# EveryVoiceTTS/FastSpeech2_lightning

Hardware: AMD Instinct MI355X
Metric: mel-frames/sec (train fwd+bwd+optimizer, whole job) (higher is better)
Workload: dtype f32

## Files before the change

### fastspeech2_lightning_amd/csrc/gemm.hip

```cpp
#include <cstdlib>

#include <string.h>

#include "gemm_common.h"

namespace {

constexpr int BK = 16;
constexpr int LDS_PAD = 4;

template <int BM, int BN>
struct Tile {
  static constexpr int TM = BM / 64;
  static constexpr int TN = BN / 64;
  static constexpr int LDA = BM + LDS_PAD;
  static constexpr int LDB = BN + LDS_PAD;
  static constexpr int A_F4 = BM * BK / 4 / 256;
  static constexpr int B_F4 = BN * BK / 4 / 256;
};

template <int ROWS, int NF4>
__device__ __forceinline__ void load_tile(float4 (&reg)[NF4], const float* __restrict__ src, int ld,
                                          bool kcontig, int row0, int nrows, int k0, int klimit,
                                          int shift, int T, bool shift_rows, bool shift_k, int tid) {
// ... 237 lines not shown
      p.Rper = a.R / a.taps;
      if (a.Mc % a.T) return FS2HIP_EINVAL;
    } else {
      if (a.a_kcontig || a.b_kcontig || a.R % a.T) return FS2HIP_EINVAL;
    }
  }
  if (a.splitk > 1 && (a.a_kcontig || a.b_kcontig || !a.workspace)) return FS2HIP_EINVAL;
  if (a.colsum && (a.a_kcontig || a.b_kcontig)) return FS2HIP_EINVAL;
  if (a.splitk <= 1) a.counters = nullptr;
  if (a.counters && (long long)a.taps * ((a.Mc + 63) / 64) * ((a.Nc + 63) / 64) > FS2_SPLITK_COUNTERS) return FS2HIP_EINVAL;
  if (a.epi == FS2_EPI_RESID && !a.resid) return FS2HIP_EINVAL;
  if (a.epi == FS2_EPI_DACT && !a.aux) return FS2HIP_EINVAL;
  {
    auto fits = [&](long long ld) { return 4LL * a.Mc * ld < 0x7fffffffLL; };
    if (!fits(a.splitk > 1 ? a.Nc : a.ldc) || (a.out_pre && !fits(a.ldpre)) ||
        (a.epi == FS2_EPI_RESID && !fits(a.ldr)) || (a.epi == FS2_EPI_DACT && !fits(a.ldaux)))
      return FS2HIP_EINVAL;
  }
  p.drop = fs2_make_drop(a.drop_p, a.drop_seed, a.drop_step);
  int chunk = (a.R + a.splitk - 1) / a.splitk;
  p.r_chunk = ((chunk + BK - 1) / BK) * BK;
  const int nz = (a.shift_operand == 1 ? a.taps : 1) * a.splitk;
  static const int env_tile = getenv("FS2_GEMM_TILE") ? atoi(getenv("FS2_GEMM_TILE")) : 0;
  int tile = a.tile ? a.tile : env_tile;
  const bool v2_ok = a.a_kcontig || !a.b_kcontig;
  const bool v1_ok = !(a.taps > 1 && a.shift_operand == 0 && (p.Rper % BK));
  if (tile == 0) {
    const bool narrow = a.Nc <= 64 || (a.Nc % 128 != 0 && a.Nc % 128 <= 64) ||
                        ((long long)((a.Mc + 127) / 128) * ((a.Nc + 127) / 128) * nz < 384);
    const bool odd_taps = a.taps > 1 && (a.shift_operand == 0 ? (p.Rper % 32) != 0 : a.T < 32);
    tile = v2_ok ? (odd_taps ? (v1_ok && !a.operand_bf16 && !a.colsum ? 3 : 7) : (narrow ? 5 : 4)) : (narrow ? 2 : 1);
  }
  if (a.operand_bf16 == 3 && (tile < 4 || tile > 9)) return FS2HIP_EINVAL;
  if (tile >= 4) {
    if (tile != 32 && !v2_ok) return FS2HIP_EINVAL;
    route = {ROUTE_V2, tile, nz};
    return 0;
  }
  if (!v1_ok || a.colsum) return FS2HIP_EINVAL;
  route = {ROUTE_V1, tile, nz};
  return 0;
}

int gemm_launch(GemmP& p, const GemmRoute& route, hipStream_t s) {
  const Fs2GemmArgs& a = p.a;
  const int tile = route.tile, nz = route.nz;
  if (route.core == ROUTE_B) {
    if (tile == 33) return fs2_gemmws4_launch(p, s);
    if (tile >= 30) return fs2_gemmws_launch(p, tile, s);
    return fs2_gemmb_launch(p, tile, nz, s);
  }
  if (route.core == ROUTE_V2) {
    if (tile == 32) return fs2_gemmws32_launch(p, s);
    return tile >= 10 ? fs2_gemm2p_launch(p, tile, nz, s) : fs2_gemm2_launch(p, tile, nz, s);
  }
  if (tile == 3) {
    p.tiles_n = (a.Nc + 63) / 64;
    dim3 grid(((a.Mc + 63) / 64) * p.tiles_n, 1, nz);
    gemm_kernel<64, 64><<<grid, dim3(256), 0, s>>>(p);
  } else if (tile == 2) {
    p.tiles_n = (a.Nc + 63) / 64;
    dim3 grid(((a.Mc + 127) / 128) * p.tiles_n, 1, nz);
    gemm_kernel<128, 64><<<grid, dim3(256), 0, s>>>(p);
  } else {
    p.tiles_n = (a.Nc + 127) / 128;
    dim3 grid(((a.Mc + 127) / 128) * p.tiles_n, 1, nz);
    gemm_kernel<128, 128><<<grid, dim3(256), 0, s>>>(p);
  }
  FS2_LAUNCH_CHECK();
  return 0;
}
}

extern "C" int fs2hip_gemm(const Fs2GemmArgs* args, void* stream) {
  if (!args) return FS2HIP_EINVAL;
  GemmP p;
  GemmRoute route;
  const int rc = gemm_prepare(args, p, route);
  if (rc != 0) return rc;
  return gemm_launch(p, route, (hipStream_t)stream);
}

extern "C" int fs2hip_gemm_grouped(const Fs2GemmArgs* args, int n, void* stream) {
  if (!args || n < 1 || n > FS2_GEMM_GROUP_MAX) return FS2HIP_EINVAL;
  if (n == 1) return fs2hip_gemm(args, stream);
  GemmPG g;
  memset(&g, 0, sizeof(g));
  g.n = n;
  const bool stored = args[0].operand_bf16 == 4;
  int tile = args[0].tile;
  if (tile == 0) tile = stored ? 23 : 7;
  for (int i = 0; i < n; ++i) {
    Fs2GemmArgs m = args[i];
    if (m.operand_bf16 != args[0].operand_bf16 || (m.operand_bf16 != 0 && m.operand_bf16 != 4)) return FS2HIP_EINVAL;
    if ((m.a_kcontig != 0) != (args[0].a_kcontig != 0) || (m.b_kcontig != 0) != (args[0].b_kcontig != 0)) return FS2HIP_EINVAL;
    if (m.taps > 1 || m.counters || m.drop_p > 0.f) return FS2HIP_EINVAL;
    m.tile = tile;
    GemmRoute route;
    const int rc = gemm_prepare(&m, g.m[i], route);
    if (rc != 0) return rc;
    if (route.core != (stored ? ROUTE_B : ROUTE_V2) || route.tile != tile || route.nz != g.m[i].a.splitk) return FS2HIP_EINVAL;
  }
  return stored ? fs2_gemmb_launch_grouped(g, tile, (hipStream_t)stream) : fs2_gemm2_launch_grouped(g, tile, (hipStream_t)stream);
}
```

### fastspeech2_lightning_amd/csrc/gemm2.hip

```cpp
#include "gemm2_core.h"
namespace {

template <int BM, int BN, bool AKC, bool BKC, int NST, int TAPS, int BF>
__device__ __forceinline__ void gemm2_body(const GemmP& p, const int bid, const int nblk) {
  constexpr int TM = BM / 64, TN = BN / 64;
  constexpr int A_TILE = BM * BK2, B_TILE = BN * BK2, STAGE = A_TILE + B_TILE;
  constexpr int L = BM / 32 + BN / 32;
  static_assert(NST >= 2 && NST <= 4 && (NST - 2) * L < 64, "ring depth");
  __shared__ __attribute__((aligned(16))) float lds[NST * STAGE];
  const Fs2GemmArgs& a = p.a;
  const int tid = threadIdx.x, lane = tid & 63;
  const int wave = __builtin_amdgcn_readfirstlane(tid >> 6);
  const int wm = wave >> 1, wn = wave & 1;
  const int ntile = p.tiles_m * p.tiles_n;
  const int unit = fs2_xcd_remap(bid, nblk);
  const int z = unit / ntile;
  const int wg = unit - z * ntile;
  const int tile_m = wg / p.tiles_n, tile_n = wg - tile_m * p.tiles_n;
  const int m0 = tile_m * BM, n0 = tile_n * BN;

  int tapz = 0, split = 0;
  if (a.shift_operand == 1 || a.splitk > 1) {
    const int ntap = a.shift_operand == 1 ? a.taps : 1;
    split = z / ntap;
// ... 108 lines not shown
      else return FS2HIP_EINVAL;
    } else if (mode == TAPS_RED) FS2_GO(true, true, TAPS_RED);
    else if (mode == TAPS_NONE) FS2_GO(true, true, TAPS_NONE);
    else return FS2HIP_EINVAL;
  } else if (a.a_kcontig && !a.b_kcontig) {
    if (mode == TAPS_RED) FS2_GO(true, false, TAPS_RED);
    else if (mode == TAPS_NONE) FS2_GO(true, false, TAPS_NONE);
    else return FS2HIP_EINVAL;
  } else if (!a.a_kcontig && !a.b_kcontig) {
    if (mode == TAPS_ROWS) FS2_GO(false, false, TAPS_ROWS);
    else if (mode == TAPS_NONE) FS2_GO(false, false, TAPS_NONE);
    else return FS2HIP_EINVAL;
  } else {
    return FS2HIP_EINVAL;
  }
  FS2_LAUNCH_CHECK();
  return 0;
}

#undef FS2_GO

template <int BM, int BN, int NST>
int launch_grouped(GemmPG& g, hipStream_t s) {
  long long total = 0;
  for (int i = 0; i < g.n; ++i) {
    GemmP& p = g.m[i];
    const Fs2GemmArgs& a = p.a;
    const int chunk = (a.R + a.splitk - 1) / a.splitk;
    p.r_chunk = ((chunk + BK2 - 1) / BK2) * BK2;
    p.tiles_m = (a.Mc + BM - 1) / BM;
    p.tiles_n = (a.Nc + BN - 1) / BN;
    if (!fs2_gemm2_offsets_fit(a)) return FS2HIP_EINVAL;
    g.start[i] = (int)total;
    total += (long long)p.tiles_m * p.tiles_n * a.splitk;
    if (total > 0x7fffffffLL) return FS2HIP_EINVAL;
  }
  for (int i = g.n; i <= FS2_GEMM_GROUP_MAX; ++i) g.start[i] = (int)total;
  const Fs2GemmArgs& a = g.m[0].a;
  dim3 grid((unsigned)total), block(256);
  if (a.a_kcontig && a.b_kcontig) gemm2g_kernel<BM, BN, true, true, NST><<<grid, block, 0, s>>>(g);
  else if (a.a_kcontig && !a.b_kcontig) gemm2g_kernel<BM, BN, true, false, NST><<<grid, block, 0, s>>>(g);
  else if (!a.a_kcontig && !a.b_kcontig) gemm2g_kernel<BM, BN, false, false, NST><<<grid, block, 0, s>>>(g);
  else return FS2HIP_EINVAL;
  FS2_LAUNCH_CHECK();
  return 0;
}

}

int fs2_gemm2_launch_grouped(GemmPG& g, int tile, hipStream_t s) {
  switch (tile) {
    case 7: return launch_grouped<64, 64, 2>(g, s);
    case 8: return launch_grouped<128, 64, 2>(g, s);
    default: return FS2HIP_EINVAL;
  }
}

int fs2_gemm2_launch(GemmP& p, int tile, int nz, hipStream_t s) {
  const Fs2GemmArgs& a = p.a;
  const int chunk = (a.R + a.splitk - 1) / a.splitk;
  p.r_chunk = ((chunk + BK2 - 1) / BK2) * BK2;
  if (!fs2_gemm2_offsets_fit(a)) return FS2HIP_EINVAL;
  switch (tile) {
    case 4: return launch_tile<128, 128, 3, false>(p, nz, s);
    case 5: return launch_tile<128, 64, 3, false>(p, nz, s);
    case 6: return launch_tile<64, 64, 4, false>(p, nz, s);
    case 7: return launch_tile<64, 64, 2, true>(p, nz, s);
    case 8: return launch_tile<128, 64, 2, false>(p, nz, s);
    case 9: return launch_tile<128, 128, 2, false>(p, nz, s);
    default: return FS2HIP_EINVAL;
  }
}
```

### fastspeech2_lightning_amd/csrc/gemm_common.h

```cpp
#pragma once
#include "common.h"

struct GemmP {
  Fs2GemmArgs a;
  int Rper;
  int tiles_m;
  int tiles_n;
  int r_chunk;
  int probe;
  int staged;
  Fs2Drop drop;
};

struct GemmPG {
  int n;
  int start[FS2_GEMM_GROUP_MAX + 1];
  GemmP m[FS2_GEMM_GROUP_MAX];
};
__device__ __forceinline__ int fs2_group_member(const GemmPG& g, int bid) {
  int i = 0;
#pragma unroll
  for (int k = 1; k < FS2_GEMM_GROUP_MAX; ++k) i += (k < g.n && bid >= g.start[k]) ? 1 : 0;
  return i;
}

constexpr int FS2_EPI_OOB = (int)0x80000000;

__device__ __forceinline__ __amdgpu_buffer_rsrc_t fs2_epi_rsrc(const float* base, int rows, int ld) {
  return __builtin_amdgcn_make_buffer_rsrc((void*)base, 0, rows * ld * 4, 0x00020000);
}
__device__ __forceinline__ float fs2_buf_load(__amdgpu_buffer_rsrc_t r, int voff, int soff) {
  return __builtin_bit_cast(float, __builtin_amdgcn_raw_buffer_load_b32(r, voff, soff, 0));
}
__device__ __forceinline__ void fs2_buf_store(__amdgpu_buffer_rsrc_t r, int voff, int soff, float v) {
  __builtin_amdgcn_raw_buffer_store_b32(__builtin_bit_cast(unsigned, v), r, voff, soff, 0);
}
constexpr int FS2_SC1 = 16;
__device__ __forceinline__ void fs2_buf_store_sc1(__amdgpu_buffer_rsrc_t r, int voff, int soff, float v) {
  __builtin_amdgcn_raw_buffer_store_b32(__builtin_bit_cast(unsigned, v), r, voff, soff, FS2_SC1);
}

template <int BM, int BN, int EPI>
__device__ __forceinline__ void gemm_epilogue_impl(const GemmP& p, const f32x16 (&acc)[BM / 64][BN / 64], float* C,
                                                   int ldc, int m0, int n0, int wm, int wn, int lane) {
  constexpr int TM = BM / 64, TN = BN / 64;
  const Fs2GemmArgs& a = p.a;
  const Fs2Drop drop = fs2_resolve_drop(p.drop);
  const int mrow = m0 + wm * (BM / 2) + 4 * (lane >> 5);
  const __amdgpu_buffer_rsrc_t rc = fs2_epi_rsrc(C, a.Mc, ldc);
#define FS2_ROWOFF(i, r) ((i) * 32 + ((r) & 3) + 8 * ((r) >> 2))
#pragma unroll
  for (int j = 0; j < TN; ++j) {
    const int n = n0 + wn * (BN / 2) + j * 32 + (lane & 31);
    const bool col = n < a.Nc;
    const float bias = (EPI >= 0 && a.bias && col) ? a.bias[n] : 0.f;
    const int vc = col ? (mrow * ldc + n) * 4 : FS2_EPI_OOB;
#pragma unroll
    for (int i = 0; i < TM; ++i) {
      float v[16];
#pragma unroll
      for (int r = 0; r < 16; ++r) v[r] = acc[i][j][r];
      if (EPI >= 0) {
#pragma unroll
        for (int r = 0; r < 16; ++r) v[r] = a.alpha * v[r] + bias;
      }
      if (EPI == FS2_EPI_ACT) {
        if (a.out_pre) {
          const __amdgpu_buffer_rsrc_t rp = fs2_epi_rsrc(a.out_pre, a.Mc, a.ldpre);
          const int vp = col ? (mrow * a.ldpre + n) * 4 : FS2_EPI_OOB;
#pragma unroll
          for (int r = 0; r < 16; ++r) fs2_buf_store(rp, vp, FS2_ROWOFF(i, r) * a.ldpre * 4, v[r]);
        }
        if (a.act == FS2_ACT_RELU) {
#pragma unroll
          for (int r = 0; r < 16; ++r) v[r] = fs2_act(FS2_ACT_RELU, v[r]);
        } else if (a.act == FS2_ACT_SILU) {
#pragma unroll
          for (int r = 0; r < 16; ++r) v[r] = fs2_act(FS2_ACT_SILU, v[r]);
        } else if (a.act == FS2_ACT_TANH) {
#pragma unroll
          for (int r = 0; r < 16; ++r) v[r] = fs2_act(FS2_ACT_TANH, v[r]);
        }
      } else if (EPI == FS2_EPI_DACT) {
        const __amdgpu_buffer_rsrc_t rx = fs2_epi_rsrc(a.aux, a.Mc, a.ldaux);
        const int vx = col ? (mrow * a.ldaux + n) * 4 : FS2_EPI_OOB;
        float x[16];
#pragma unroll
        for (int r = 0; r < 16; ++r) x[r] = fs2_buf_load(rx, vx, FS2_ROWOFF(i, r) * a.ldaux * 4);
        if (a.act == FS2_ACT_RELU) {
#pragma unroll
          for (int r = 0; r < 16; ++r) v[r] *= fs2_dact(FS2_ACT_RELU, x[r]);
        } else if (a.act == FS2_ACT_SILU) {
#pragma unroll
          for (int r = 0; r < 16; ++r) v[r] *= fs2_dact(FS2_ACT_SILU, x[r]);
        } else if (a.act == FS2_ACT_TANH) {
#pragma unroll
          for (int r = 0; r < 16; ++r) v[r] *= fs2_dact(FS2_ACT_TANH, x[r]);
        }
      }
      if (EPI > 0 && drop.on) {
        if ((ldc & 1) == 0) {
          const int par = lane & 1;
          const unsigned he = (unsigned)((mrow * ldc + n) + par * ldc);
          const unsigned sh = par << 4;
#pragma unroll
          for (int r = 0; r < 16; r += 2) {
            const uint32_t H = fs2_hash32_lo(drop.seed, (he + (unsigned)(FS2_ROWOFF(i, r) * ldc)) >> 1);
            const uint32_t Hn = (uint32_t)__builtin_amdgcn_mov_dpp((int)H, 0xB1, 0xF, 0xF, true);
            const uint32_t ha = par ? Hn : H, hb = par ? H : Hn;
            v[r] *= ((ha >> sh) & 0xffffu) < drop.thresh ? 0.f : drop.scale;
            v[r + 1] *= ((hb >> sh) & 0xffffu) < drop.thresh ? 0.f : drop.scale;
          }
        } else {
#pragma unroll
          for (int r = 0; r < 16; ++r)
            v[r] *= fs2_drop_factor(drop, (unsigned long long)((unsigned)(vc + FS2_ROWOFF(i, r) * ldc * 4) >> 2));
        }
      }
      if (EPI == FS2_EPI_RESID) {
        const __amdgpu_buffer_rsrc_t rx = fs2_epi_rsrc(a.resid, a.Mc, a.ldr);
        const int vx = col ? (mrow * a.ldr + n) * 4 : FS2_EPI_OOB;
        float x[16];
#pragma unroll
        for (int r = 0; r < 16; ++r) x[r] = fs2_buf_load(rx, vx, FS2_ROWOFF(i, r) * a.ldr * 4);
#pragma unroll
        for (int r = 0; r < 16; ++r) v[r] = x[r] + a.res_scale * v[r];
      }
      if (EPI == -2) {
#pragma unroll
        for (int r = 0; r < 16; ++r) fs2_buf_store_sc1(rc, vc, FS2_ROWOFF(i, r) * ldc * 4, v[r]);
      } else {
#pragma unroll
        for (int r = 0; r < 16; ++r) fs2_buf_store(rc, vc, FS2_ROWOFF(i, r) * ldc * 4, v[r]);
      }
    }
  }
#undef FS2_ROWOFF
}

template <int BM, int BN>
__device__ __forceinline__ void splitk_finish(const GemmP& p, int m0, int n0, int tapz) {
  const Fs2GemmArgs& a = p.a;
  __shared__ int last_one;
  const int slot = (tapz * ((a.Mc + BM - 1) / BM) + m0 / BM) * p.tiles_n + n0 / BN;
  asm volatile("s_waitcnt vmcnt(0)" ::: "memory");
  __syncthreads();
  if (threadIdx.x == 0)
    last_one = __hip_atomic_fetch_add(a.counters + slot, 1, __ATOMIC_RELAXED, __HIP_MEMORY_SCOPE_AGENT) == a.splitk - 1;
  __syncthreads();
  if (!last_one) return;
  const long long slab = (long long)a.Mc * a.Nc;
  const long long kstride = (long long)a.taps * slab;
  const __amdgpu_buffer_rsrc_t rw = __builtin_amdgcn_make_buffer_rsrc((void*)(a.workspace + (long long)tapz * slab), 0, 0x7ffffffc, 0x00020000);
  float* C = a.C + (a.shift_operand == 1 ? (long long)tapz * a.c_tap_stride : 0);
  const bool vec = (a.Nc % 4) == 0 && (a.ldc % 4) == 0 && ((uintptr_t)C % 16) == 0 && ((uintptr_t)a.workspace % 16) == 0;
  constexpr int C4 = BN / 4;
  for (int e = threadIdx.x; e < BM * C4; e += blockDim.x) {
    const int m = m0 + e / C4, n = n0 + (e % C4) * 4;
    if (m >= a.Mc || n >= a.Nc) continue;
    const int off = (m * a.Nc + n) * 4;
    if (vec) {
      f32x4 t = {0.f, 0.f, 0.f, 0.f};
      for (int k0 = 0; k0 < a.splitk; k0 += 8) {
        f32x4 v[8];
#pragma unroll
        for (int u = 0; u < 8; ++u) {
          const __amdgpu_buffer_rsrc_t rk = __builtin_amdgcn_make_buffer_rsrc(
              (void*)(a.workspace + (long long)tapz * slab + (k0 + u) * kstride), 0, k0 + u < a.splitk ? 0x7ffffffc : 0, 0x00020000);
          v[u] = __builtin_bit_cast(f32x4, __builtin_amdgcn_raw_buffer_load_b128(rk, off, 0, FS2_SC1));
        }
        if (k0 == 0) {
          t = v[0];
#pragma unroll
          for (int u = 1; u < 8; ++u)
            if (u < a.splitk) t += v[u];
        } else {
#pragma unroll
          for (int u = 0; u < 8; ++u)
            if (k0 + u < a.splitk) t += v[u];
        }
      }
      *reinterpret_cast<f32x4*>(C + (long long)m * a.ldc + n) = t;
    } else {
      for (int i = 0; i < 4 && n + i < a.Nc; ++i) {
        float t = __builtin_bit_cast(float, __builtin_amdgcn_raw_buffer_load_b32(rw, off + 4 * i, 0, FS2_SC1));
        for (int k = 1; k < a.splitk; ++k) {
          const __amdgpu_buffer_rsrc_t rk = __builtin_amdgcn_make_buffer_rsrc(
              (void*)(a.workspace + (long long)tapz * slab + k * kstride), 0, 0x7ffffffc, 0x00020000);
          t += __builtin_bit_cast(float, __builtin_amdgcn_raw_buffer_load_b32(rk, off + 4 * i, 0, FS2_SC1));
        }
        C[(long long)m * a.ldc + n + i] = t;
      }
    }
  }
  if (threadIdx.x == 0) __hip_atomic_store(a.counters + slot, 0, __ATOMIC_RELAXED, __HIP_MEMORY_SCOPE_AGENT);
}

template <int BM, int BN>
__device__ __forceinline__ void gemm_epilogue(const GemmP& p, const f32x16 (&acc)[BM / 64][BN / 64], int m0, int n0,
                                              int wm, int wn, int lane, int split, int tapz) {
  const Fs2GemmArgs& a = p.a;
  float* C = a.C;
  if (a.splitk > 1) {
    C = a.workspace + ((long long)split * a.taps + tapz) * ((long long)a.Mc * a.Nc);
    if (a.counters) {
      gemm_epilogue_impl<BM, BN, -2>(p, acc, C, a.Nc, m0, n0, wm, wn, lane);
      splitk_finish<BM, BN>(p, m0, n0, tapz);
    } else {
      gemm_epilogue_impl<BM, BN, -1>(p, acc, C, a.Nc, m0, n0, wm, wn, lane);
    }
    return;
  }
  if (a.shift_operand == 1) C += (long long)tapz * a.c_tap_stride;
  switch (a.epi) {
    case FS2_EPI_ACT: gemm_epilogue_impl<BM, BN, FS2_EPI_ACT>(p, acc, C, a.ldc, m0, n0, wm, wn, lane); break;
    case FS2_EPI_RESID: gemm_epilogue_impl<BM, BN, FS2_EPI_RESID>(p, acc, C, a.ldc, m0, n0, wm, wn, lane); break;
    case FS2_EPI_DACT: gemm_epilogue_impl<BM, BN, FS2_EPI_DACT>(p, acc, C, a.ldc, m0, n0, wm, wn, lane); break;
    default: gemm_epilogue_impl<BM, BN, 0>(p, acc, C, a.ldc, m0, n0, wm, wn, lane); break;
  }
}

__device__ __forceinline__ int fs2_xcd_remap(int orig, int nwg) {
  const int q = nwg >> 3, r = nwg & 7, xcd = orig & 7;
  return (xcd < r ? xcd * (q + 1) : r * (q + 1) + (xcd - r) * q) + (orig >> 3);
}

int fs2_gemm2_launch(GemmP& p, int tile, int nz, hipStream_t s);
int fs2_gemm2p_launch(GemmP& p, int tile, int nz, hipStream_t s);
int fs2_gemmb_launch(GemmP& p, int tile, int nz, hipStream_t s);
int fs2_gemmws_launch(GemmP& p, int tile, hipStream_t s);
int fs2_gemmws32_launch(GemmP& p, hipStream_t s);
int fs2_gemmws4_launch(GemmP& p, hipStream_t s);
int fs2_gemm2_launch_grouped(GemmPG& g, int tile, hipStream_t s);
int fs2_gemmb_launch_grouped(GemmPG& g, int tile, hipStream_t s);
int fs2_tail_fixup(const float* ws, int S, long long slab, float* C, int ldc, const float* bias, float alpha, int m0,
                   int Mc, int Nc, hipStream_t s);
```

### fastspeech2_lightning_amd/hip.py

```python
from __future__ import annotations

import ctypes as C
import os
import time
from pathlib import Path
from typing import Optional

os.environ.setdefault("GPU_MAX_HW_QUEUES", "8")

import torch

_LIB_PATH = Path(__file__).resolve().parent / "_fs2hip.so"
_lib = None

ACT_NONE, ACT_RELU, ACT_SILU, ACT_TANH = 0, 1, 2, 3
EPI_STORE, EPI_ACT, EPI_RESID, EPI_DACT = 0, 1, 2, 3
_ACT = {None: 0, "none": 0, "relu": 1, "silu": 2, "tanh": 3}


class GemmArgs(C.Structure):
    _fields_ = [
        ("A", C.c_void_p), ("B", C.c_void_p), ("C", C.c_void_p),
        ("Mc", C.c_int), ("Nc", C.c_int), ("R", C.c_int),
        ("lda", C.c_int), ("ldb", C.c_int), ("ldc", C.c_int),
# ... 242 lines not shown
HYBRID_WS_FLOATS = 512 * 128 * 128


def reserve_workspace(n: int, device) -> torch.Tensor:
    key = (device.index if isinstance(device, torch.device) else device, _stream())
    ws = _WS.get(key)
    if ws is None or ws.numel() < n:
        dev = device if isinstance(device, torch.device) else torch.device("cuda", device)
        ws = torch.empty(max(n, 1 << 22), device=dev, dtype=torch.float32)
        _WS[key] = ws
    return ws


def _workspace(n: int, device) -> torch.Tensor:
    return reserve_workspace(n, device)


SPLITK_COUNTERS = 4096
SPLITK_IN_KERNEL = os.environ.get("FS2_SPLITK_IN_KERNEL", "0") != "0"
SPLITK_MAX = int(os.environ.get("FS2_SPLITK_MAX", 16))
_COUNTERS = {}


def splitk_counters(device) -> torch.Tensor:
    key = (device.index if isinstance(device, torch.device) else device, _stream())
    c = _COUNTERS.get(key)
    if c is None:
        dev = device if isinstance(device, torch.device) else torch.device("cuda", device)
        c = _COUNTERS[key] = torch.zeros(SPLITK_COUNTERS, device=dev, dtype=torch.int32)
    return c


GEMM_PROFILE = None


GEMM_TUNE = os.environ.get("FS2_GEMM_TUNE", "1") != "0"
GEMM_BF16 = 0
BF16_STORAGE = os.environ.get("FS2_BF16_STORAGE", "1") != "0"
PRECISIONS = {"32-true": 0, "32": 0, "fp32": 0, "bf16-mixed": 1, "bf16": 1, "32-split": 2}


def set_precision(precision) -> None:
    global GEMM_BF16
    key = str(precision)
    _req(key in PRECISIONS, f"precision must be one of {sorted(PRECISIONS)}, got {precision!r}")
    GEMM_BF16 = PRECISIONS[key]


def get_precision() -> str:
    return {0: "32-true", 1: "bf16-mixed", 2: "32-split"}[int(GEMM_BF16)]


GEMM_TILES_B = (20, 21, 22, 23, 24, 25, 26, 30, 31, 33)
GEMM_TILES = (1, 2, 3, 4, 5, 6, 7, 8, 9, 10, 11, 12, 13, 14, 15, 32)
_EXCLUDED = {int(t) for t in os.environ.get("FS2_GEMM_EXCLUDE_TILES", "").split(",") if t.strip()}
if _EXCLUDED:
    GEMM_TILES_B = tuple(t for t in GEMM_TILES_B if t not in _EXCLUDED)
    GEMM_TILES = tuple(t for t in GEMM_TILES if t not in _EXCLUDED)
_TILE_CACHE = {}
TILE_GEN = [0]
_TILE_TIMINGS = {}
_TILE_CALLS = {}


def refine_tiles_in_step(step, rounds: int = 5, candidates: int = 2, top: int = 16, min_gain: float = 0.004,
                         log=None, settle=None, count_step=None, agree=None, timer=None, deadline=None):
    def out_of_time():
        if deadline is None:
            return False
        late = float(time.perf_counter() > deadline)
        return (agree(late) if agree is not None else late) > 0

    def event_timer(fn, n):
        torch.cuda.synchronize()
        e0, e1 = torch.cuda.Event(enable_timing=True), torch.cuda.Event(enable_timing=True)
        e0.record()
        for _ in range(n):
            fn()
        e1.record()
        e1.synchronize()
        return e0.elapsed_time(e1) / n

    def timed():
        if settle is not None:
            settle()
        t = (timer or event_timer)(step, rounds)
        return agree(t) if agree is not None else t

    for v in _TILE_CALLS.values():
        v[0] = 0
    (count_step or step)()
    base = min(timed(), timed())
    order = sorted((k for k in _TILE_TIMINGS if _TILE_CALLS.get(k, [0])[0] > 0),
                   key=lambda k: -_TILE_TIMINGS[k][0][0] * _TILE_CALLS[k][0])[:top]
    changed = 0
    for key in order:
        if out_of_time():
            break
        keep = _TILE_CACHE[key]
        for ms_iso, tile in _TILE_TIMINGS[key][1:1 + candidates]:
            if out_of_time():
                break
            _TILE_CACHE[key] = tile
            TILE_GEN[0] += 1
            t = min(timed(), timed())
            if t < base * (1.0 - min_gain):
                if log:
# ... 59 lines not shown
        if k == "__format__":
            continue
        if k == "__groups__":
            for gk, gv in v.items():
                _GROUP_TILE_CACHE[ast.literal_eval(gk)] = int(gv)
            continue
        _TILE_CACHE[ast.literal_eval(k) if isinstance(k, str) else tuple(k)] = int(v)
    TILE_GEN[0] += 1


def save_tile_cache(path) -> None:
    import json
    Path(path).write_text(json.dumps(tile_table(), indent=0, sort_keys=True))


def load_tile_cache(path) -> bool:
    import json
    pth = Path(path)
    if not pth.exists():
        return False
    load_tile_table(json.loads(pth.read_text()))
    return True


_TILE_CACHE_ENV_LOADED = False


def _tune_tile(a) -> int:
    global _TILE_CACHE_ENV_LOADED
    if not _TILE_CACHE_ENV_LOADED:
        _TILE_CACHE_ENV_LOADED = True
        if os.environ.get("FS2_GEMM_TILE_CACHE"):
            load_tile_cache(os.environ["FS2_GEMM_TILE_CACHE"])
    if not GEMM_TUNE and not _TILE_CACHE:
        return 0
    key = _tile_key(a)
    t = _TILE_CACHE.get(key)
    if t is not None:
        c = _TILE_CALLS.get(key)
        if c is not None:
            c[0] += 1
        return t
    if not GEMM_TUNE or _REC is not None or torch.cuda.is_current_stream_capturing():
        return 0
    L, s = real_lib(), _stream()
    best, best_ms = 0, float("inf")
    timings = []
    order = sorted(GEMM_TILES, key=lambda t: (t < 4, t)) if a.operand_bf16 else GEMM_TILES
    if a.operand_bf16 == 4:
        order = GEMM_TILES_B
    for tile in order:
        if a.operand_bf16 and tile < 4 and best:
            break
        a.tile = tile
        rc = L.fs2hip_gemm(C.byref(a), s)
        if rc == -22:
            continue
        _ok(rc, "gemm")
        ms = float("inf")
        for _ in range(2):
            e0, e1 = torch.cuda.Event(enable_timing=True), torch.cuda.Event(enable_timing=True)
            e0.record()
            for _ in range(4):
                _ok(L.fs2hip_gemm(C.byref(a), s), "gemm")
            e1.record()
            e1.synchronize()
            ms = min(ms, e0.elapsed_time(e1))
        timings.append((ms, tile))
        if ms < best_ms:
            best, best_ms = tile, ms
    _TILE_CACHE[key] = best
    TILE_GEN[0] += 1
    if timings:
        _TILE_TIMINGS[key] = sorted(timings)
        _TILE_CALLS[key] = [1]
    return best


_TILE_REFUSED = set()


def _refusal_key(a):
    return (a.tile, a.Mc, a.Nc, a.R, a.T, a.taps, a.lda, a.ldb, a.ldc, a.epi, a.io_bf16, a.operand_bf16, a.splitk,
            bool(a.colsum), (a.C or 0) % 16)


def _launch_gemm(a):
    if a.tile != 0 and _TILE_REFUSED and _refusal_key(a) in _TILE_REFUSED:
        a.tile = 0
    rc = lib().fs2hip_gemm(C.byref(a), _stream())
    if rc == -22 and a.tile != 0:
        _TILE_REFUSED.add(_refusal_key(a))
        a.tile = 0
        rc = lib().fs2hip_gemm(C.byref(a), _stream())
    _ok(rc, "gemm")


def _gemm(_algorithmic=True, **kw):
    a = GemmArgs()
    a.taps, a.alpha, a.res_scale, a.splitk = 1, 1.0, 1.0, 1
    for k, v in kw.items():
        setattr(a, k, v)
    if not a.workspace:
        ws = _workspace(HYBRID_WS_FLOATS, _current_device())
        a.workspace, a.workspace_floats = _p(ws), ws.numel()
    if not a.operand_bf16:
        a.operand_bf16 = int(GEMM_BF16) if _algorithmic else 0
    a.tile = _tune_tile(a)
    if _GROUP is not None:
        _GROUP.entries.append((a, _algorithmic, _stream()))
        return
    if GEMM_PROFILE is None or not _algorithmic:
        _launch_gemm(a)
        return
    e0, e1 = torch.cuda.Event(enable_timing=True), torch.cuda.Event(enable_timing=True)
    e0.record()
    _launch_gemm(a)
    e1.record()
    _profile_gemm(a, e0, e1)


def _gemm_cost(a):
    ntap = a.taps if a.shift_operand == 1 else 1
    ra = a.R // a.taps if (a.taps > 1 and a.shift_operand == 0) else a.R
    esz = 2.0 if a.operand_bf16 >= 3 else 4.0
    osz = 2.0 if (a.io_bf16 & 1) else 4.0
    nbytes = (esz * (a.Mc * ra + a.Nc * a.R) + osz * a.Mc * a.Nc * ntap + 4.0 * (a.Mc * a.Nc if a.resid else 0)
              + (2.0 if (a.io_bf16 & 2) else 4.0) * (a.Mc * a.Nc if a.aux else 0) + osz * (a.Mc * a.Nc if a.out_pre else 0))
    return 2.0 * a.Mc * a.Nc * a.R * ntap, nbytes


def _profile_gemm(a, e0, e1, members=None):
    ntap = a.taps if a.shift_operand == 1 else 1
    flops, nbytes = _gemm_cost(a)
    kind = (a.a_kcontig, a.b_kcontig, a.taps, a.shift_operand, a.splitk, a.epi, a.tile)
    if members:
        cost = [_gemm_cost(m) for m in members]
        flops, nbytes = sum(c[0] for c in cost), sum(c[1] for c in cost)
        kind += ("grouped", len(members))
    GEMM_PROFILE.append((e0, e1, flops, a.Mc, a.Nc, a.R * ntap, nbytes, kind))


GEMM_GROUP = os.environ.get("FS2_GEMM_GROUP", "1") != "0"
GROUP_MAX = 8
GROUP_TILES = {0: (7, 8), 4: (23, 26, 22)}
_GROUP = None
_GROUP_TILE_CACHE = {}
GROUP_STATS = {"launches": 0, "members": 0, "single": 0}


class gemm_group:

    def __enter__(self):
        global _GROUP
        self.entries, self.after, self.outer = [], [], True
        if GEMM_GROUP and _GROUP is None:
            _GROUP = self
        else:
            self.outer = False
        return self

    def __exit__(self, et, ev, tb):
        global _GROUP
        if not self.outer:
            return False
        _GROUP = None
        if et is None:
            _launch_group(self.entries)
            for fn in self.after:
                fn()
        return False


def _group_class(a):
    if a.taps > 1 or a.counters or a.drop_p > 0 or a.operand_bf16 not in GROUP_TILES:
        return None
    return (a.operand_bf16, bool(a.a_kcontig), bool(a.b_kcontig))


def _group_tile(arr, n, members, stream):
    tiles = GROUP_TILES[members[0].operand_bf16]
    if not GEMM_TUNE and not _TILE_CACHE:
        return 0
    key = tuple(_tile_key(m) for m in members)
    t = _GROUP_TILE_CACHE.get(key)
    if t is not None:
        return t
    if not GEMM_TUNE or _REC is not None or torch.cuda.is_current_stream_capturing():
        common = {m.tile for m in members}
        return common.pop() if len(common) == 1 and members[0].tile in tiles else 0
    L, best, best_ms = real_lib(), 0, float("inf")
    for tile in tiles:
        arr[0].tile = tile
        if L.fs2hip_gemm_grouped(arr, n, stream) != 0:
            continue
        ms = float("inf")
        for _ in range(2):
            e0, e1 = torch.cuda.Event(enable_timing=True), torch.cuda.Event(enable_timing=True)
# ... 1352 lines not shown
```

Before: 951,900.

## Add 16x16 MFMA GEMM kernel with 80-wide tiles for non-64-multiple shapes

Adds a new f32 GEMM variant (tile 16) that uses 16x16x4 MFMA instructions with 128x80 or 80x128 block tiles. It is chosen only when a dimension is not a multiple of 64 and an 80-wide tile wastes less padding than a 64-wide one (e.g. 80 mel bins). The epilogue is generalised over accumulator geometry so both layouts share one code path. The autotuner and the grouped launcher now consider the new tile, at the cost of more kernel instantiations and extra tuning time.

```diff
diff --git a/fastspeech2_lightning_amd/csrc/gemm.hip b/fastspeech2_lightning_amd/csrc/gemm.hip
--- a/fastspeech2_lightning_amd/csrc/gemm.hip
+++ b/fastspeech2_lightning_amd/csrc/gemm.hip
@@ -313,6 +313,7 @@
   }
   if (route.core == ROUTE_V2) {
     if (tile == 32) return fs2_gemmws32_launch(p, s);
+    if (tile == 16) return fs2_gemm2n_launch(p, nz, s);
     return tile >= 10 ? fs2_gemm2p_launch(p, tile, nz, s) : fs2_gemm2_launch(p, tile, nz, s);
   }
   if (tile == 3) {
diff --git a/fastspeech2_lightning_amd/csrc/gemm2.hip b/fastspeech2_lightning_amd/csrc/gemm2.hip
--- a/fastspeech2_lightning_amd/csrc/gemm2.hip
+++ b/fastspeech2_lightning_amd/csrc/gemm2.hip
@@ -184,6 +184,7 @@
   switch (tile) {
     case 7: return launch_grouped<64, 64, 2>(g, s);
     case 8: return launch_grouped<128, 64, 2>(g, s);
+    case 16: return fs2_gemm2n_launch_grouped(g, s);
     default: return FS2HIP_EINVAL;
   }
 }
diff --git a/fastspeech2_lightning_amd/csrc/gemm2n.hip b/fastspeech2_lightning_amd/csrc/gemm2n.hip
--- /dev/null
+++ b/fastspeech2_lightning_amd/csrc/gemm2n.hip
@@ -0,0 +1,253 @@
+#include "gemm2_core.h"
+namespace {
+
+constexpr int pad32(int rows) { return (rows + 31) / 32 * 32; }
+
+template <int ROWS, bool KC>
+struct RdAddr16 {
+  unsigned g[KC ? 2 : 1];
+  __device__ __forceinline__ void setup(int wrow0, int r, int q) {
+    if (KC) {
+#pragma unroll
+      for (int G = 0; G < 2; ++G) g[G] = ((wrow0 + r) * BK2 + (((4 * G + q) ^ ((r >> 1) & 7)) << 2)) * 4;
+    } else {
+      g[0] = (4 * q * ROWS + wrow0 + r) * 4;
+    }
+  }
+};
+
+template <int G, int I, int ROWS, int T, bool KC>
+__device__ __forceinline__ void frag16_read(Frag<T, KC>& f, const RdAddr16<ROWS, KC>& ra, unsigned base) {
+  if constexpr (I < T) {
+    if constexpr (KC) {
+      lds_rd128<I * 16 * BK2 * 4>(f.q[I], ra.g[G] + base);
+    } else {
+      lds_rd32<((16 * G + 0) * ROWS + 16 * I) * 4>(f.q[I][0], ra.g[0] + base);
+      lds_rd32<((16 * G + 1) * ROWS + 16 * I) * 4>(f.q[I][1], ra.g[0] + base);
+      lds_rd32<((16 * G + 2) * ROWS + 16 * I) * 4>(f.q[I][2], ra.g[0] + base);
+      lds_rd32<((16 * G + 3) * ROWS + 16 * I) * 4>(f.q[I][3], ra.g[0] + base);
+    }
+    frag16_read<G, I + 1, ROWS, T, KC>(f, ra, base);
+  }
+}
+
+template <int BM, int BN, int WM, int WN, bool AKC, bool BKC, int NST, int TAPS>
+__device__ __forceinline__ void gemm2n_body(const GemmP& p, const int bid, const int nblk) {
+  typedef Geo16<BM, BN, WM, WN> G;
+  constexpr int TMB = G::TMB, TNB = G::TNB;
+  constexpr int AROWS = pad32(BM), BROWS = pad32(BN);
+  constexpr int A_TILE = AROWS * BK2, B_TILE = BROWS * BK2, STAGE = A_TILE + B_TILE;
+  constexpr int L = AROWS / 32 + BROWS / 32;
+  static_assert(WM * WN == 4 && NST >= 2 && NST <= 3 && (NST - 2) * L < 64, "geometry");
+  __shared__ __attribute__((aligned(16))) float lds[NST * STAGE];
+  const Fs2GemmArgs& a = p.a;
+  const int tid = threadIdx.x, lane = tid & 63;
+  const int wave = __builtin_amdgcn_readfirstlane(tid >> 6);
+  const int wm = WM == 4 ? wave : 0, wn = WN == 4 ? wave : 0;
+  const int ntile = p.tiles_m * p.tiles_n;
+  const int unit = fs2_xcd_remap(bid, nblk);
+  const int z = unit / ntile;
+  const int wg = unit - z * ntile;
+  const int tile_m = wg / p.tiles_n, tile_n = wg - tile_m * p.tiles_n;
+  const int m0 = tile_m * BM, n0 = tile_n * BN;
+
+  int tapz = 0, split = 0;
+  if (a.shift_operand == 1 || a.splitk > 1) {
+    const int ntap = a.shift_operand == 1 ? a.taps : 1;
+    split = z / ntap;
+    tapz = z - split * ntap;
+  }
+  const int r_begin = split * p.r_chunk;
+  const int r_end = min(a.R, r_begin + p.r_chunk);
+  const int nkt = (r_end - r_begin + BK2 - 1) / BK2;
+  const int shift_z = tapz * a.tap_mul + a.tap_add;
+
+  f32x4 acc[TMB][TNB];
+#pragma unroll
+  for (int i = 0; i < TMB; ++i)
+#pragma unroll
+    for (int j = 0; j < TNB; ++j) acc[i][j] = f32x4{0.f, 0.f, 0.f, 0.f};
+
+  Pieces<AROWS> pa;
+  Pieces<BROWS> pb;
+  Stream<AKC, BKC, TAPS> st;
+  setup_pieces<AROWS, AKC, true, TAPS>(pa, p, m0, r_begin, tid);
+  setup_pieces<BROWS, BKC, false, TAPS>(pb, p, n0, r_begin, tid);
+  if constexpr (AROWS != BM) {
+#pragma unroll
+    for (int it = 0; it < AROWS / 32; ++it) {
+      const int pidx = it * 256 + tid;
+      const int row = AKC ? (pidx >> 3) : (pidx % (AROWS / 4)) * 4;
+      if (row >= BM) pa.voff[it] = FS2_OOB;
+    }
+  }
+  if constexpr (BROWS != BN) {
+#pragma unroll
+    for (int it = 0; it < BROWS / 32; ++it) {
+      const int pidx = it * 256 + tid;
+      const int row = BKC ? (pidx >> 3) : (pidx % (BROWS / 4)) * 4;
+      if (row >= BN) pb.voff[it] = FS2_OOB;
+    }
+  }
+  st.begin(p, r_begin, r_end, shift_z);
+  auto issue = [&](int stage) {
+    float* At = lds + stage * STAGE;
+    st.template issue<AROWS, BROWS>(p, At, At + A_TILE, pa, pb, wave, tid);
+  };
+
+  const int r16 = lane & 15, q = lane >> 4;
+  const unsigned lds0 = (unsigned)(unsigned long long)(__attribute__((address_space(3))) float*)lds;
+  RdAddr16<AROWS, AKC> rda;
+  RdAddr16<BROWS, BKC> rdb;
+  rda.setup(wm * (BM / WM), r16, q);
+  rdb.setup(wn * (BN / WN), r16, q);
+
+  float cs[TMB];
+#pragma unroll
+  for (int i = 0; i < TMB; ++i) cs[i] = 0.f;
+  const bool do_cs = !AKC && !BKC && a.colsum != nullptr && tile_n == 0 && tapz == 0 && wn == 0;
+
+  for (int kt = 0; kt < NST - 1 && kt < nkt; ++kt) issue(kt);
+  int stage = 0;
+  for (int kt = 0; kt < nkt; ++kt) {
+    const int newer = min(NST - 2, nkt - 1 - kt);
+    if (NST >= 3 && newer == 1) wait_vmcnt_barrier<L>();
+    else wait_vmcnt_barrier<0>();
+    if (kt + NST - 1 < nkt) issue(stage == 0 ? NST - 1 : stage - 1);
+    const unsigned sa = lds0 + stage * (STAGE * 4), sb = sa + A_TILE * 4;
+    Frag<TMB, AKC> fa[2];
+    Frag<TNB, BKC> fb[2];
+    frag16_read<0, 0, AROWS>(fa[0], rda, sa);
+    frag16_read<0, 0, BROWS>(fb[0], rdb, sb);
+    frag16_read<1, 0, AROWS>(fa[1], rda, sa);
+    frag16_read<1, 0, BROWS>(fb[1], rdb, sb);
+    constexpr int RD = Frag<TMB, AKC>::READS + Frag<TNB, BKC>::READS;
+#pragma unroll
+    for (int g = 0; g < 2; ++g) {
+      if (g == 0) lds_wait<RD>();
+      else lds_wait<0>();
+      fa[g].pin_all();
+      fb[g].pin_all();
+      if (!AKC && do_cs) {
+#pragma unroll
+        for (int i = 0; i < TMB; ++i) cs[i] += (fa[g].get(i, 0) + fa[g].get(i, 1)) + (fa[g].get(i, 2) + fa[g].get(i, 3));
+      }
+#pragma unroll
+      for (int j = 0; j < 4; ++j)
+#pragma unroll
+        for (int i = 0; i < TMB; ++i)
+#pragma unroll
+          for (int jn = 0; jn < TNB; ++jn)
+            acc[i][jn] = __builtin_amdgcn_mfma_f32_16x16x4f32(fa[g].get(i, j), fb[g].get(jn, j), acc[i][jn], 0, 0, 0);
+    }
+    stage = stage + 1 == NST ? 0 : stage + 1;
+  }
+  gemm_epilogue<BM, BN, G>(p, acc, m0, n0, wm, wn, lane, split, tapz);
+  if (do_cs) {
+#pragma unroll
+    for (int i = 0; i < TMB; ++i) {
+      float t = cs[i] + __shfl_xor(cs[i], 16, 64);
+      t += __shfl_xor(t, 32, 64);
+      const int m = m0 + wm * (BM / WM) + 16 * i + lane;
+      if (lane < 16 && m < a.Mc) a.colsum[(long long)split * a.Mc + m] = t;
+    }
+  }
+}
+
+template <int BM, int BN, int WM, int WN, bool AKC, bool BKC, int NST, int TAPS>
+__global__ __launch_bounds__(256) void gemm2n_kernel(GemmP p) {
+  gemm2n_body<BM, BN, WM, WN, AKC, BKC, NST, TAPS>(p, blockIdx.x, gridDim.x);
+}
+
+template <int BM, int BN, int WM, int WN, bool AKC, bool BKC, int NST>
+__global__ __launch_bounds__(256) void gemm2ng_kernel(GemmPG g) {
+  const int i = fs2_group_member(g, blockIdx.x);
+  gemm2n_body<BM, BN, WM, WN, AKC, BKC, NST, TAPS_NONE>(g.m[i], blockIdx.x - g.start[i], g.start[i + 1] - g.start[i]);
+}
+
+constexpr int NST_N = 3;
+
+inline int form_of(const Fs2GemmArgs& a) {
+  auto pays = [](int n) { return n % 64 != 0 && (n + 79) / 80 * 80 < (n + 63) / 64 * 64; };
+  if (pays(a.Nc)) return 1;
+  if (pays(a.Mc) && !a.a_kcontig) return 2;
+  return 0;
+}
+
+template <int BM, int BN, int WM, int WN>
+int launch_form(GemmP& p, int nz, hipStream_t s) {
+  const Fs2GemmArgs& a = p.a;
+  p.tiles_m = (a.Mc + BM - 1) / BM;
+  p.tiles_n = (a.Nc + BN - 1) / BN;
+  if ((long long)p.tiles_m * p.tiles_n * nz > 0x7fffffffLL) return FS2HIP_EINVAL;
+  dim3 grid(p.tiles_m * p.tiles_n * nz), block(256);
+  int mode = TAPS_NONE;
+  if (a.taps > 1) {
+    if (a.shift_operand == 0) mode = (p.Rper % BK2 == 0) ? TAPS_RED : TAPS_GENERIC;
+    else mode = a.T >= BK2 ? TAPS_ROWS : TAPS_GENERIC;
+  }
+  if (mode == TAPS_GENERIC) return FS2HIP_EINVAL;
+  if (a.a_kcontig && a.b_kcontig) {
+    if constexpr (WM == 4) {
+      if (mode == TAPS_RED) gemm2n_kernel<BM, BN, WM, WN, true, true, NST_N, TAPS_RED><<<grid, block, 0, s>>>(p);
+      else if (mode == TAPS_NONE) gemm2n_kernel<BM, BN, WM, WN, true, true, NST_N, TAPS_NONE><<<grid, block, 0, s>>>(p);
+      else return FS2HIP_EINVAL;
+    } else return FS2HIP_EINVAL;
+  } else if (a.a_kcontig && !a.b_kcontig) {
+    if constexpr (WM == 4) {
+      if (mode == TAPS_RED) gemm2n_kernel<BM, BN, WM, WN, true, false, NST_N, TAPS_RED><<<grid, block, 0, s>>>(p);
+      else if (mode == TAPS_NONE) gemm2n_kernel<BM, BN, WM, WN, true, false, NST_N, TAPS_NONE><<<grid, block, 0, s>>>(p);
+      else return FS2HIP_EINVAL;
+    } else return FS2HIP_EINVAL;
+  } else if (!a.a_kcontig && !a.b_kcontig) {
+    if (mode == TAPS_ROWS) gemm2n_kernel<BM, BN, WM, WN, false, false, NST_N, TAPS_ROWS><<<grid, block, 0, s>>>(p);
+    else if (mode == TAPS_NONE) gemm2n_kernel<BM, BN, WM, WN, false, false, NST_N, TAPS_NONE><<<grid, block, 0, s>>>(p);
+    else return FS2HIP_EINVAL;
+  } else {
+    return FS2HIP_EINVAL;
+  }
+  FS2_LAUNCH_CHECK();
+  return 0;
+}
+
+}
+
+int fs2_gemm2n_launch(GemmP& p, int nz, hipStream_t s) {
+  const Fs2GemmArgs& a = p.a;
+  if (a.operand_bf16) return FS2HIP_EINVAL;
+  const int chunk = (a.R + a.splitk - 1) / a.splitk;
+  p.r_chunk = ((chunk + BK2 - 1) / BK2) * BK2;
+  if (!fs2_gemm2_offsets_fit(a)) return FS2HIP_EINVAL;
+  switch (form_of(a)) {
+    case 1: return launch_form<128, 80, 4, 1>(p, nz, s);
+    case 2: return launch_form<80, 128, 1, 4>(p, nz, s);
+    default: return FS2HIP_EINVAL;
+  }
+}
+
+int fs2_gemm2n_launch_grouped(GemmPG& g, hipStream_t s) {
+  constexpr int BM = 128, BN = 80;
+  long long total = 0;
+  for (int i = 0; i < g.n; ++i) {
+    GemmP& p = g.m[i];
+    const Fs2GemmArgs& a = p.a;
+    if (a.operand_bf16 || form_of(a) != 1) return FS2HIP_EINVAL;
+    const int chunk = (a.R + a.splitk - 1) / a.splitk;
+    p.r_chunk = ((chunk + BK2 - 1) / BK2) * BK2;
+    p.tiles_m = (a.Mc + BM - 1) / BM;
+    p.tiles_n = (a.Nc + BN - 1) / BN;
+    if (!fs2_gemm2_offsets_fit(a)) return FS2HIP_EINVAL;
+    g.start[i] = (int)total;
+    total += (long long)p.tiles_m * p.tiles_n * a.splitk;
+    if (total > 0x7fffffffLL) return FS2HIP_EINVAL;
+  }
+  for (int i = g.n; i <= FS2_GEMM_GROUP_MAX; ++i) g.start[i] = (int)total;
+  const Fs2GemmArgs& a = g.m[0].a;
+  dim3 grid((unsigned)total), block(256);
+  if (a.a_kcontig && a.b_kcontig) gemm2ng_kernel<BM, BN, 4, 1, true, true, NST_N><<<grid, block, 0, s>>>(g);
+  else if (a.a_kcontig && !a.b_kcontig) gemm2ng_kernel<BM, BN, 4, 1, true, false, NST_N><<<grid, block, 0, s>>>(g);
+  else if (!a.a_kcontig && !a.b_kcontig) gemm2ng_kernel<BM, BN, 4, 1, false, false, NST_N><<<grid, block, 0, s>>>(g);
+  else return FS2HIP_EINVAL;
+  FS2_LAUNCH_CHECK();
+  return 0;
+}
diff --git a/fastspeech2_lightning_amd/csrc/gemm_common.h b/fastspeech2_lightning_amd/csrc/gemm_common.h
--- a/fastspeech2_lightning_amd/csrc/gemm_common.h
+++ b/fastspeech2_lightning_amd/csrc/gemm_common.h
@@ -40,62 +40,82 @@
   __builtin_amdgcn_raw_buffer_store_b32(__builtin_bit_cast(unsigned, v), r, voff, soff, FS2_SC1);
 }
 
-template <int BM, int BN, int EPI>
-__device__ __forceinline__ void gemm_epilogue_impl(const GemmP& p, const f32x16 (&acc)[BM / 64][BN / 64], float* C,
+template <int BM, int BN>
+struct Geo32 {
+  static constexpr int TM = BM / 64, TN = BN / 64, NV = 16;
+  typedef f32x16 Acc[TM][TN];
+  static __device__ __forceinline__ int mrow(int m0, int wm, int lane) { return m0 + wm * (BM / 2) + 4 * (lane >> 5); }
+  static __device__ __forceinline__ int ncol(int n0, int wn, int j, int lane) { return n0 + wn * (BN / 2) + j * 32 + (lane & 31); }
+  static constexpr int rowoff(int i, int r) { return i * 32 + (r & 3) + 8 * (r >> 2); }
+  static __device__ __forceinline__ float val(const Acc& acc, int i, int j, int r) { return acc[i][j][r]; }
+};
+template <int BM, int BN, int WM, int WN>
+struct Geo16 {
+  static constexpr int TMB = BM / WM / 16, TNB = BN / WN / 16;
+  static constexpr int TM = 1, TN = TNB, NV = 4 * TMB;
+  typedef f32x4 Acc[TMB][TNB];
+  static __device__ __forceinline__ int mrow(int m0, int wm, int lane) { return m0 + wm * (BM / WM) + 4 * (lane >> 4); }
+  static __device__ __forceinline__ int ncol(int n0, int wn, int j, int lane) { return n0 + wn * (BN / WN) + j * 16 + (lane & 15); }
+  static constexpr int rowoff(int i, int r) { return 16 * (r >> 2) + (r & 3); }
+  static __device__ __forceinline__ float val(const Acc& acc, int i, int j, int r) { return acc[r >> 2][j][r & 3]; }
+};
+
+template <int BM, int BN, int EPI, class G = Geo32<BM, BN>>
+__device__ __forceinline__ void gemm_epilogue_impl(const GemmP& p, const typename G::Acc& acc, float* C,
                                                    int ldc, int m0, int n0, int wm, int wn, int lane) {
-  constexpr int TM = BM / 64, TN = BN / 64;
+  constexpr int TM = G::TM, TN = G::TN, NV = G::NV;
   const Fs2GemmArgs& a = p.a;
   const Fs2Drop drop = fs2_resolve_drop(p.drop);
-  const int mrow = m0 + wm * (BM / 2) + 4 * (lane >> 5);
+  const int mrow = G::mrow(m0, wm, lane);
   const __amdgpu_buffer_rsrc_t rc = fs2_epi_rsrc(C, a.Mc, ldc);
-#define FS2_ROWOFF(i, r) ((i) * 32 + ((r) & 3) + 8 * ((r) >> 2))
+#define FS2_ROWOFF(i, r) (G::rowoff(i, r))
 #pragma unroll
   for (int j = 0; j < TN; ++j) {
-    const int n = n0 + wn * (BN / 2) + j * 32 + (lane & 31);
+    const int n = G::ncol(n0, wn, j, lane);
     const bool col = n < a.Nc;
     const float bias = (EPI >= 0 && a.bias && col) ? a.bias[n] : 0.f;
     const int vc = col ? (mrow * ldc + n) * 4 : FS2_EPI_OOB;
 #pragma unroll
     for (int i = 0; i < TM; ++i) {
-      float v[16];
-#pragma unroll
-      for (int r = 0; r < 16; ++r) v[r] = acc[i][j][r];
+      float v[NV];
+#pragma unroll
+      for (int r = 0; r < NV; ++r) v[r] = G::val(acc, i, j, r);
       if (EPI >= 0) {
 #pragma unroll
-        for (int r = 0; r < 16; ++r) v[r] = a.alpha * v[r] + bias;
+        for (int r = 0; r < NV; ++r) v[r] = a.alpha * v[r] + bias;
       }
       if (EPI == FS2_EPI_ACT) {
         if (a.out_pre) {
           const __amdgpu_buffer_rsrc_t rp = fs2_epi_rsrc(a.out_pre, a.Mc, a.ldpre);
           const int vp = col ? (mrow * a.ldpre + n) * 4 : FS2_EPI_OOB;
 #pragma unroll
-          for (int r = 0; r < 16; ++r) fs2_buf_store(rp, vp, FS2_ROWOFF(i, r) * a.ldpre * 4, v[r]);
+          for (int r = 0; r < NV; ++r) fs2_buf_store(rp, vp, FS2_ROWOFF(i, r) * a.ldpre * 4, v[r]);
         }
         if (a.act == FS2_ACT_RELU) {
 #pragma unroll
-          for (int r = 0; r < 16; ++r) v[r] = fs2_act(FS2_ACT_RELU, v[r]);
+          for (int r = 0; r < NV; ++r) v[r] = fs2_act(FS2_ACT_RELU, v[r]);
         } else if (a.act == FS2_ACT_SILU) {
 #pragma unroll
-          for (int r = 0; r < 16; ++r) v[r] = fs2_act(FS2_ACT_SILU, v[r]);
+          for (int r = 0; r < NV; ++r) v[r] = fs2_act(FS2_ACT_SILU, v[r]);
         } else if (a.act == FS2_ACT_TANH) {
 #pragma unroll
-          for (int r = 0; r < 16; ++r) v[r] = fs2_act(FS2_ACT_TANH, v[r]);
+          for (int r = 0; r < NV; ++r) v[r] = fs2_act(FS2_ACT_TANH, v[r]);
         }
       } else if (EPI == FS2_EPI_DACT) {
         const __amdgpu_buffer_rsrc_t rx = fs2_epi_rsrc(a.aux, a.Mc, a.ldaux);
         const int vx = col ? (mrow * a.ldaux + n) * 4 : FS2_EPI_OOB;
-        float x[16];
-#pragma unroll
-        for (int r = 0; r < 16; ++r) x[r] = fs2_buf_load(rx, vx, FS2_ROWOFF(i, r) * a.ldaux * 4);
+        float x[NV];
+#pragma unroll
+        for (int r = 0; r < NV; ++r) x[r] = fs2_buf_load(rx, vx, FS2_ROWOFF(i, r) * a.ldaux * 4);
         if (a.act == FS2_ACT_RELU) {
 #pragma unroll
-          for (int r = 0; r < 16; ++r) v[r] *= fs2_dact(FS2_ACT_RELU, x[r]);
+          for (int r = 0; r < NV; ++r) v[r] *= fs2_dact(FS2_ACT_RELU, x[r]);
         } else if (a.act == FS2_ACT_SILU) {
 #pragma unroll
-          for (int r = 0; r < 16; ++r) v[r] *= fs2_dact(FS2_ACT_SILU, x[r]);
+          for (int r = 0; r < NV; ++r) v[r] *= fs2_dact(FS2_ACT_SILU, x[r]);
         } else if (a.act == FS2_ACT_TANH) {
 #pragma unroll
-          for (int r = 0; r < 16; ++r) v[r] *= fs2_dact(FS2_ACT_TANH, x[r]);
+          for (int r = 0; r < NV; ++r) v[r] *= fs2_dact(FS2_ACT_TANH, x[r]);
         }
       }
       if (EPI > 0 && drop.on) {
@@ -104,7 +124,7 @@
           const unsigned he = (unsigned)((mrow * ldc + n) + par * ldc);
           const unsigned sh = par << 4;
 #pragma unroll
-          for (int r = 0; r < 16; r += 2) {
+          for (int r = 0; r < NV; r += 2) {
             const uint32_t H = fs2_hash32_lo(drop.seed, (he + (unsigned)(FS2_ROWOFF(i, r) * ldc)) >> 1);
             const uint32_t Hn = (uint32_t)__builtin_amdgcn_mov_dpp((int)H, 0xB1, 0xF, 0xF, true);
             const uint32_t ha = par ? Hn : H, hb = par ? H : Hn;
@@ -113,25 +133,25 @@
           }
         } else {
 #pragma unroll
-          for (int r = 0; r < 16; ++r)
+          for (int r = 0; r < NV; ++r)
             v[r] *= fs2_drop_factor(drop, (unsigned long long)((unsigned)(vc + FS2_ROWOFF(i, r) * ldc * 4) >> 2));
         }
       }
       if (EPI == FS2_EPI_RESID) {
         const __amdgpu_buffer_rsrc_t rx = fs2_epi_rsrc(a.resid, a.Mc, a.ldr);
         const int vx = col ? (mrow * a.ldr + n) * 4 : FS2_EPI_OOB;
-        float x[16];
-#pragma unroll
-        for (int r = 0; r < 16; ++r) x[r] = fs2_buf_load(rx, vx, FS2_ROWOFF(i, r) * a.ldr * 4);
-#pragma unroll
-        for (int r = 0; r < 16; ++r) v[r] = x[r] + a.res_scale * v[r];
+        float x[NV];
+#pragma unroll
+        for (int r = 0; r < NV; ++r) x[r] = fs2_buf_load(rx, vx, FS2_ROWOFF(i, r) * a.ldr * 4);
+#pragma unroll
+        for (int r = 0; r < NV; ++r) v[r] = x[r] + a.res_scale * v[r];
       }
       if (EPI == -2) {
 #pragma unroll
-        for (int r = 0; r < 16; ++r) fs2_buf_store_sc1(rc, vc, FS2_ROWOFF(i, r) * ldc * 4, v[r]);
+        for (int r = 0; r < NV; ++r) fs2_buf_store_sc1(rc, vc, FS2_ROWOFF(i, r) * ldc * 4, v[r]);
       } else {
 #pragma unroll
-        for (int r = 0; r < 16; ++r) fs2_buf_store(rc, vc, FS2_ROWOFF(i, r) * ldc * 4, v[r]);
+        for (int r = 0; r < NV; ++r) fs2_buf_store(rc, vc, FS2_ROWOFF(i, r) * ldc * 4, v[r]);
       }
     }
   }
@@ -196,27 +216,27 @@
   if (threadIdx.x == 0) __hip_atomic_store(a.counters + slot, 0, __ATOMIC_RELAXED, __HIP_MEMORY_SCOPE_AGENT);
 }
 
-template <int BM, int BN>
-__device__ __forceinline__ void gemm_epilogue(const GemmP& p, const f32x16 (&acc)[BM / 64][BN / 64], int m0, int n0,
+template <int BM, int BN, class G = Geo32<BM, BN>>
+__device__ __forceinline__ void gemm_epilogue(const GemmP& p, const typename G::Acc& acc, int m0, int n0,
                                               int wm, int wn, int lane, int split, int tapz) {
   const Fs2GemmArgs& a = p.a;
   float* C = a.C;
   if (a.splitk > 1) {
     C = a.workspace + ((long long)split * a.taps + tapz) * ((long long)a.Mc * a.Nc);
     if (a.counters) {
-      gemm_epilogue_impl<BM, BN, -2>(p, acc, C, a.Nc, m0, n0, wm, wn, lane);
+      gemm_epilogue_impl<BM, BN, -2, G>(p, acc, C, a.Nc, m0, n0, wm, wn, lane);
       splitk_finish<BM, BN>(p, m0, n0, tapz);
     } else {
-      gemm_epilogue_impl<BM, BN, -1>(p, acc, C, a.Nc, m0, n0, wm, wn, lane);
+      gemm_epilogue_impl<BM, BN, -1, G>(p, acc, C, a.Nc, m0, n0, wm, wn, lane);
     }
     return;
   }
   if (a.shift_operand == 1) C += (long long)tapz * a.c_tap_stride;
   switch (a.epi) {
-    case FS2_EPI_ACT: gemm_epilogue_impl<BM, BN, FS2_EPI_ACT>(p, acc, C, a.ldc, m0, n0, wm, wn, lane); break;
-    case FS2_EPI_RESID: gemm_epilogue_impl<BM, BN, FS2_EPI_RESID>(p, acc, C, a.ldc, m0, n0, wm, wn, lane); break;
-    case FS2_EPI_DACT: gemm_epilogue_impl<BM, BN, FS2_EPI_DACT>(p, acc, C, a.ldc, m0, n0, wm, wn, lane); break;
-    default: gemm_epilogue_impl<BM, BN, 0>(p, acc, C, a.ldc, m0, n0, wm, wn, lane); break;
+    case FS2_EPI_ACT: gemm_epilogue_impl<BM, BN, FS2_EPI_ACT, G>(p, acc, C, a.ldc, m0, n0, wm, wn, lane); break;
+    case FS2_EPI_RESID: gemm_epilogue_impl<BM, BN, FS2_EPI_RESID, G>(p, acc, C, a.ldc, m0, n0, wm, wn, lane); break;
+    case FS2_EPI_DACT: gemm_epilogue_impl<BM, BN, FS2_EPI_DACT, G>(p, acc, C, a.ldc, m0, n0, wm, wn, lane); break;
+    default: gemm_epilogue_impl<BM, BN, 0, G>(p, acc, C, a.ldc, m0, n0, wm, wn, lane); break;
   }
 }
 
@@ -227,6 +247,8 @@
 
 int fs2_gemm2_launch(GemmP& p, int tile, int nz, hipStream_t s);
 int fs2_gemm2p_launch(GemmP& p, int tile, int nz, hipStream_t s);
+int fs2_gemm2n_launch(GemmP& p, int nz, hipStream_t s);
+int fs2_gemm2n_launch_grouped(GemmPG& g, hipStream_t s);
 int fs2_gemmb_launch(GemmP& p, int tile, int nz, hipStream_t s);
 int fs2_gemmws_launch(GemmP& p, int tile, hipStream_t s);
 int fs2_gemmws32_launch(GemmP& p, hipStream_t s);
diff --git a/fastspeech2_lightning_amd/hip.py b/fastspeech2_lightning_amd/hip.py
--- a/fastspeech2_lightning_amd/hip.py
+++ b/fastspeech2_lightning_amd/hip.py
@@ -318,7 +318,7 @@
 
 
 GEMM_TILES_B = (20, 21, 22, 23, 24, 25, 26, 30, 31, 33)
-GEMM_TILES = (1, 2, 3, 4, 5, 6, 7, 8, 9, 10, 11, 12, 13, 14, 15, 32)
+GEMM_TILES = (1, 2, 3, 4, 5, 6, 7, 8, 9, 10, 11, 12, 13, 14, 15, 16, 32)
 _EXCLUDED = {int(t) for t in os.environ.get("FS2_GEMM_EXCLUDE_TILES", "").split(",") if t.strip()}
 if _EXCLUDED:
     GEMM_TILES_B = tuple(t for t in GEMM_TILES_B if t not in _EXCLUDED)
@@ -484,6 +484,8 @@
     for tile in order:
         if a.operand_bf16 and tile < 4 and best:
             break
+        if tile == 16 and (a.operand_bf16 or (a.Mc % 64 == 0 and a.Nc % 64 == 0)):
+            continue
         a.tile = tile
         rc = L.fs2hip_gemm(C.byref(a), s)
         if rc == -22:
@@ -575,7 +577,7 @@
 
 GEMM_GROUP = os.environ.get("FS2_GEMM_GROUP", "1") != "0"
 GROUP_MAX = 8
-GROUP_TILES = {0: (7, 8), 4: (23, 26, 22)}
+GROUP_TILES = {0: (7, 8, 16), 4: (23, 26, 22)}
 _GROUP = None
 _GROUP_TILE_CACHE = {}
 GROUP_STATS = {"launches": 0, "members": 0, "single": 0}
```

After: 951,400. About the same (-0.0%).
